# guzba/zippy

Measured on AMD Instinct MI355X. Metric: GiB/s uncompressed throughput (compress BestSpeed + uncompress), 4096x1 MiB batch, higher is better.
Workload: dtype u8

## Files before the change

zippy_amd/csrc/zh_l1_match.hip:

```cpp
#include <cstdlib>
#include <cstring>

#include "zh_common.h"
#include "zh_kprof.h"
#include "zh_tables.h"

namespace {
constexpr uint32_t kHashMul = 0x1e35a7bdu;
constexpr uint32_t kCntWords = 1024;
struct __attribute__((packed)) Bytes16 {
  uint32_t x, y, z, w;
};

}

template <bool kLdsTable>
__global__ __launch_bounds__(64) void zh_l1_match_kernel(const uint8_t* __restrict__ d_src,
                                                         ZhCompressArgs a, int huffman_only,
                                                         uint16_t* __restrict__ table_pool,
                                                         uint32_t* __restrict__ next_frag,
                                                         const uint32_t* __restrict__ order,
                                                         uint32_t* __restrict__ cost, uint32_t ticket_base) {
  __shared__ uint32_t s_hist[ZH_HIST_STRIDE];
  __shared__ uint32_t s_scr[kCntWords];
  __shared__ uint32_t s_bits[512];
  __shared__ uint32_t s_nmatch;
  uint32_t* const s_cover = s_scr;

  const unsigned lane = zh_lane();
  __shared__ uint16_t s_table_lds[kLdsTable ? 16384 : 2];
  uint16_t* const s_table = kLdsTable ? s_table_lds : table_pool + (size_t)blockIdx.x * 16384u;
  uint32_t taken = 0;
  for (uint32_t ticket = ticket_base + blockIdx.x; ticket < a.nfrags; taken++) {
  const uint32_t f = order ? order[ticket] : ticket;
  const uint64_t t_start = zh_clock();
  KPROF_DECL(16);
  const ZhFragDesc fd = a.frags[f];
  const uint32_t n = fd.len;
  const uint8_t* src = d_src + fd.src_off;
  uint16_t* m_pos = a.m_pos + (size_t)f * ZH_MAX_MATCHES_PER_FRAG;
  uint16_t* m_len = a.m_len + (size_t)f * ZH_MAX_MATCHES_PER_FRAG;
  uint16_t* m_off = a.m_off + (size_t)f * ZH_MAX_MATCHES_PER_FRAG;

  const uint32_t mis = (uint32_t)((uintptr_t)src & 3u);
  const uint32_t* asrc = reinterpret_cast<const uint32_t*>(src - mis);
  const uint32_t last_dw = n ? (n + mis - 1u) >> 2 : 0u;
  auto dw = [&](uint32_t i) -> uint32_t { return asrc[i < last_dw ? i : last_dw]; };
  auto ld32 = [&](uint32_t p) -> uint32_t {
    const uint32_t q = p + mis, i = q >> 2;
    return __builtin_amdgcn_alignbyte(dw(i + 1), dw(i), q);
  };
  for (uint32_t i = lane; i < ZH_HIST_STRIDE; i += 64) s_hist[i] = 0;
  for (uint32_t i = lane; i < kCntWords; i += 64) s_scr[i] = 0;

  uint32_t table_size = 256, shift = 24;
  while (table_size < 16384u && table_size < n) {
    table_size <<= 1;
    shift--;
  }
  const uint32_t e0 = (!huffman_only && n >= 4) ? (((ld32(0) * kHashMul) >> 17) & 1u) << 15 : 0u;
  for (uint32_t i = lane; i < 512; i += 64) s_bits[i] = 0;
  zh_wave_sync();
  KPROF_MARK(0);

  {
    uint32_t nm = 0;
    if (!huffman_only && n >= 15) {
      const uint32_t ip_limit = n - 15;
      uint32_t ip = 1;
      uint32_t K = 0;
      bool post = false;
      bool finished = false;
      while (!finished) {
        const bool dense = post || K < 32u;
        uint32_t pos, step, W0 = 0;
        if (dense) {
          W0 = post ? ip - 1u : ip;
          pos = W0 + lane;
          step = 1;
        } else {
          const uint32_t s = 32 + K, q = s >> 5, r = s & 31u, j = lane;
          uint32_t off = q * j;
          if (j > 32u - r) off += j - (32u - r);
          if (j > 64u - r) off += j - (64u - r);
          pos = ip + off;
          step = (s + j) >> 5;
        }
        const bool valid = pos + step <= ip_limit;
        if (!valid) pos = 1;
        Bytes16 av = {0, 0, 0, 0};
        if (valid) av = *reinterpret_cast<const Bytes16*>(src + pos);
        const uint32_t a0 = av.x, a1 = av.y, a2 = av.z, a3 = av.w;
        const uint32_t hp = a0 * kHashMul;
        const uint32_t h = hp >> shift, tag = (hp >> 17) & 1u;
        uint32_t oldw = e0;
        if (valid && ((s_bits[h >> 5] >> (h & 31u)) & 1u))
          oldw = kLdsTable ? (uint32_t)s_table[h]
                           : (uint32_t)__hip_atomic_load(s_table + h, __ATOMIC_RELAXED, __HIP_MEMORY_SCOPE_AGENT);
        const uint32_t old = oldw & 0x7fffu;
        const bool fetch = valid && (oldw >> 15) == tag;
        const uint32_t ck = (h & (kCntWords * 4u - 1u)) >> 2, cs = (h & 3u) * 8u;
        if (valid) atomicAdd(&s_scr[ck], 1u << cs);
        zh_wave_sync();
        Bytes16 qv = {0, 0, 0, 0};
        if (fetch) qv = *reinterpret_cast<const Bytes16*>(src + old);
        const uint32_t cnt = valid ? (s_scr[ck] >> cs) & 255u : 0u;
        zh_wave_sync();
        if (valid) s_scr[ck] = 0;
        const uint32_t x0 = fetch ? a0 ^ qv.x : 1u;
        const uint32_t x1 = a1 ^ qv.y;
        const uint32_t x2 = a2 ^ qv.z;
        const uint32_t x3 = a3 ^ qv.w;
        const uint32_t c0 = min(((uint32_t)__ffs((int)x0) - 1u) >> 3, 4u);
        const uint32_t c1 = min(((uint32_t)__ffs((int)x1) - 1u) >> 3, 4u);
        const uint32_t c2 = min(((uint32_t)__ffs((int)x2) - 1u) >> 3, 4u);
        const uint32_t c3 = min(((uint32_t)__ffs((int)x3) - 1u) >> 3, 4u);
        const uint32_t c23 = c2 + (c2 == 4u ? c3 : 0u);
        const uint32_t c123 = c1 + (c1 == 4u ? c23 : 0u);
        const uint32_t eqlen = c0 + (c0 == 4u ? c123 : 0u);

        const uint64_t V = __ballot(valid);
        const uint64_t H = __ballot(valid && x0 == 0);
        const uint64_t C = __ballot(cnt > 1u);
        uint64_t Cw = C;
        if (C && __popcll(C) <= 16) {
          Cw = 0;
          for (uint64_t cm = C; cm; cm &= cm - 1) {
            const uint32_t g = (uint32_t)__ffsll((long long)cm) - 1u;
            const uint32_t hg = __builtin_amdgcn_readlane(h, g);
            const bool same_h = valid && h == hg;
            if (__ballot(same_h) & ((1ull << g) - 1ull)) Cw |= 1ull << g;
          }
        }
        const uint32_t t = V == ~0ull ? 64u : (uint32_t)__ffsll((long long)~V) - 1u;

        KPROF_MARK(1);
        KPROF_COUNT(6, 1);
#ifndef ZH_EMU
        __builtin_amdgcn_s_setprio(1);
#endif
        uint64_t ins = post ? 1ull : 0ull;
        uint32_t i = post ? 1u : 0u;
        bool reprobe = post;
        uint32_t hop = 0x8000u;
        if (dense) {
          const uint64_t ev = (H | Cw) >> lane;
          const uint32_t d = ev ? (uint32_t)__ffsll((long long)ev) - 1u : 64u;
          const uint32_t info = eqlen | ((uint32_t)((Cw >> lane) & 1ull) << 5);
          const uint32_t gi = (uint32_t)__shfl((int)info, (int)((lane + d) & 63u), 64);
          if (d < 32u && gi < 16u) {
            const uint32_t g0 = lane + d, nx = g0 + gi;
            hop = g0 | 0x40u | (nx << 8) | ((d + 1u) << 16) | ((nx <= 64u ? nx - 1u : g0) << 22);
          } else if (!ev && lane >= 32u) {
            hop = 63u | (64u << 8);
          }
        }
        const uint32_t tt = ip_limit > W0 ? ip_limit - W0 : 0u;
        for (;;) {
          if (dense && i < 64u) {
            uint64_t sel = 0;
            uint32_t cur = zh_bcast(i), tv = 0x8000u;
            KPROF_MARK(3);
            bool go = true;
            if (!reprobe && K) {
              tv = __builtin_amdgcn_readlane(hop, cur);
              go = !(tv & 0x8000u) && (tv & 0x40u) && K + ((tv & 63u) - cur) <= 31u;
            }
            const uint32_t lim = zh_bcast(tt < 64u ? tt : 64u);
            if (go && cur < lim) {
#ifdef ZH_EMU
              do {
                tv = __builtin_amdgcn_readlane(hop, cur);
                if ((tv & 0x8040u) != 0x40u) break;
                const uint32_t g = tv & 63u, nxt = (tv >> 8) & 127u;
                sel |= 1ull << g;
                ins |= (~0ull << cur) & (~0ull >> (63u - g));
                ins |= 1ull << (nxt <= 64u ? nxt - 1u : g);
                cur = nxt;
              } while (cur < lim);
#else
              uint32_t t0, g, nxt;
              uint64_t m1;
              asm volatile(
                  "1:\n\t"
                  "v_readlane_b32 %[tv], %[hop], %[cur]\n\t"
                  "s_bitcmp1_b32 %[tv], 6\n\t"
                  "s_cbranch_scc0 2f\n\t"
                  "s_and_b32 %[g], %[tv], 63\n\t"
                  "s_bitset1_b64 %[sel], %[g]\n\t"
                  "s_bfe_u32 %[t0], %[tv], 0x60010\n\t"
                  "s_bfm_b64 %[m1], %[t0], %[cur]\n\t"
                  "s_or_b64 %[ins], %[ins], %[m1]\n\t"
                  "s_bfe_u32 %[t0], %[tv], 0x60016\n\t"
                  "s_bitset1_b64 %[ins], %[t0]\n\t"
                  "s_bfe_u32 %[cur], %[tv], 0x70008\n\t"
                  "s_cmp_lt_u32 %[cur], %[lim]\n\t"
                  "s_cbranch_scc1 1b\n\t"
                  "2:"
                  : [tv] "=&s"(tv), [cur] "+s"(cur), [sel] "+s"(sel), [ins] "+s"(ins), [t0] "=&s"(t0),
                    [g] "=&s"(g), [nxt] "=&s"(nxt), [m1] "=&s"(m1)
                  : [hop] "v"(hop), [lim] "s"(lim)
                  : "scc");
#endif
            }
            const bool chained = cur != i;
            bool run_out = false;
            if (go && cur < lim && !(tv & 0x8040u) && tt >= 64u) {
              K = (chained || reprobe ? 63u : K + 64u) - cur;
              ins |= ~0ull << cur;
              run_out = true;
            }
            KPROF_MARK(2);
            if (sel) {
              KPROF_COUNT(8, __popcll(sel));
              if ((sel >> lane) & 1ull) {
                const uint32_t k = nm + (uint32_t)__popcll(sel & zh_lanemask_lt());
                zh_store_nt(m_pos + k, (uint16_t)pos);
                zh_store_nt(m_len + k, (uint16_t)eqlen);
                zh_store_nt(m_off + k, (uint16_t)(pos - old));
              }
              nm += (uint32_t)__popcll(sel);
            }
            if (run_out) {
              post = false;
              ip = W0 + 64u;
              break;
            }
            if (chained) {
              K = 0;
              if (cur >= tt) {
                finished = true;
                break;
              }
              if (cur >= 64u) {
                post = true;
                ip = W0 + cur;
                break;
              }
              i = cur;
              reprobe = true;
            }
          }
          KPROF_COUNT(9, 1);
          if (i >= t) {
            finished = true;
            break;
          }
          uint32_t g = i;
          if (!reprobe) {
            const uint32_t last_dense = dense ? i + (31u - K) : 63u;
            uint32_t lim = last_dense < 63u ? last_dense : 63u;
            if (t - 1u < lim) lim = t - 1u;
            const uint64_t E = (H | Cw) & (~0ull << i);
            g = E ? (uint32_t)__ffsll((long long)E) - 1u : 64u;
            if (g > lim) {
              KPROF_COUNT(12, 1);
              ins |= (~0ull << i) & (~0ull >> (63u - lim));
              if (dense && lim == last_dense) {
                K = 32;
                ip = W0 + lim + 1u;
                post = false;
              } else if (lim + 1u == t && t < 64u) {
                finished = true;
              } else {
                K += 64u - i;
                post = false;
                if (dense) {
                  ip = W0 + 64u;
                } else {
                  ip = __builtin_amdgcn_readlane(pos, 63) + __builtin_amdgcn_readlane(step, 63);
                }
              }
              break;
            }
            if (g > i) ins |= (~0ull << i) & ((1ull << g) - 1ull);
            K += g - i;
          }
          uint32_t cand, flen;
          bool hit;
          if ((Cw >> g) & 1ull) {
            KPROF_COUNT(14, 1);
            const uint32_t hg = __builtin_amdgcn_readlane(h, g);
            const uint64_t same = __ballot(h == hg) & ins;
            if (same) {
              const uint32_t k = 63u - (uint32_t)__clzll((long long)same);
              cand = __builtin_amdgcn_readlane(pos, k);
              hit = __builtin_amdgcn_readlane(a0, k) == __builtin_amdgcn_readlane(a0, g);
              flen = 4;
              if (hit) {
                const uint32_t y1 = (uint32_t)__builtin_amdgcn_readlane(a1, k) ^ (uint32_t)__builtin_amdgcn_readlane(a1, g);
                if (y1) {
                  flen = 4u + (((uint32_t)__ffs((int)y1) - 1u) >> 3);
                } else {
                  const uint32_t y2 = (uint32_t)__builtin_amdgcn_readlane(a2, k) ^ (uint32_t)__builtin_amdgcn_readlane(a2, g);
                  if (y2) {
                    flen = 8u + (((uint32_t)__ffs((int)y2) - 1u) >> 3);
                  } else {
                    const uint32_t y3 = (uint32_t)__builtin_amdgcn_readlane(a3, k) ^ (uint32_t)__builtin_amdgcn_readlane(a3, g);
                    flen = y3 ? 12u + (((uint32_t)__ffs((int)y3) - 1u) >> 3) : 16u;
                  }
                }
              }
            } else {
              cand = __builtin_amdgcn_readlane(old, g);
              hit = (H >> g) & 1ull;
              flen = __builtin_amdgcn_readlane(eqlen, g);
            }
          } else {
            cand = __builtin_amdgcn_readlane(old, g);
            hit = (H >> g) & 1ull;
            flen = __builtin_amdgcn_readlane(eqlen, g);
          }
          ins |= 1ull << g;
          if (!hit) {
            if (reprobe) {
              reprobe = false;
              K = 0;
            } else {
              K++;
            }
            i = g + 1u;
            if (dense && K == 32u) {
              ip = W0 + i;
              post = false;
              break;
            }
            if (i >= 64u) {
              post = false;
              ip = dense ? W0 + 64u
                         : __builtin_amdgcn_readlane(pos, 63) + __builtin_amdgcn_readlane(step, 63);
              break;
            }
            continue;
          }
          const uint32_t mp = __builtin_amdgcn_readlane(pos, g);
          const uint32_t limit = n < mp + 258u ? n : mp + 258u;
          uint32_t matched;
          if (flen < 16u) {
            KPROF_COUNT(15, 1);
            matched = flen;
          } else {
            KPROF_COUNT(10, 1);
            zh_wave_sync();
            const uint32_t o = flen + 4u * lane;
            uint32_t avail = 0;
            if (mp + o < limit) avail = limit - (mp + o) < 4u ? limit - (mp + o) : 4u;
            const uint32_t x = ld32(mp + o) ^ ld32(cand + o);
            uint32_t eq = min(((uint32_t)__ffs((int)x) - 1u) >> 3, 4u);
            if (eq > avail) eq = avail;
            const uint64_t stop = __ballot(eq < 4u);
            const uint32_t fl = (uint32_t)__ffsll((long long)stop) - 1u;
            matched = flen + 4u * fl + __builtin_amdgcn_readlane(eq, fl);
          }
          if (matched > limit - mp) matched = limit - mp;
          if (lane == 0) {
            zh_store_nt(m_pos + nm, (uint16_t)mp);
            zh_store_nt(m_len + nm, (uint16_t)matched);
            zh_store_nt(m_off + nm, (uint16_t)(mp - cand));
          }
          nm++;
          ip = mp + matched;
          K = 0;
          post = true;
          if (ip >= ip_limit) {
            finished = true;
            break;
          }
          const uint32_t ni = g + matched;
          if (!dense || ni >= 64u) break;
          ins |= 1ull << (ni - 1u);
          i = ni;
          reprobe = true;
        }
        KPROF_MARK(3);
#ifndef ZH_EMU
        __builtin_amdgcn_s_setprio(0);
#endif
        if (finished) break;
        const bool mine = (ins >> lane) & 1ull;
        if (mine) atomicOr(&s_bits[h >> 5], 1u << (h & 31u));
        if (mine && !((C >> lane) & 1ull)) s_table[h] = (uint16_t)(pos | (tag << 15));
        uint64_t cc = ins & C;
        while (cc) {
          const uint32_t jx = (uint32_t)__ffsll((long long)cc) - 1u;
          cc &= cc - 1;
          if (lane == jx) s_table[h] = (uint16_t)(pos | (tag << 15));
        }
        zh_wave_sync();
        KPROF_MARK(4);
      }
    }
    if (lane == 0) s_nmatch = nm;
  }
  __threadfence_block();
  zh_wave_sync();
  KPROF_MARK(3);
  const uint32_t nmatch = s_nmatch;

  uint32_t extra_bits = 0, covered = 0;
  {
    const uint32_t mlast = nmatch ? nmatch - 1u : 0u;
    auto at = [&](uint32_t m) { return m < nmatch ? m : mlast; };
    uint32_t pq = m_pos[at(lane)], lq = m_len[at(lane)], oq = m_off[at(lane)];
    for (uint32_t m = lane; m - lane < nmatch; m += 64) {
      const uint32_t p = pq, l = lq, o = oq;
      pq = m_pos[at(m + 64u)];
      lq = m_len[at(m + 64u)];
      oq = m_off[at(m + 64u)];
      if (m < nmatch) {
        const uint32_t li = zh_len_code(l), di = zh_dist_code(o);
        atomicAdd(&s_hist[257 + li], 1u);
        atomicAdd(&s_hist[ZH_NUM_LITLEN + di], 1u);
        extra_bits += zh_len_extra_bits(li) + zh_dist_extra_bits(di);
        covered += l;
        atomicXor(&s_cover[(p + 1u) >> 5], 1u << ((p + 1u) & 31u));
        if (p + l < kCntWords * 32u) atomicXor(&s_cover[(p + l) >> 5], 1u << ((p + l) & 31u));
      }
    }
  }
  zh_wave_sync();
  {
    uint32_t carry = 0;
    for (uint32_t w0 = 0; w0 < kCntWords && w0 * 32u < n; w0 += 64) {
      uint32_t x = s_cover[w0 + lane];
#pragma unroll
      for (uint32_t sh = 1; sh < 32; sh <<= 1) x ^= x << sh;
      const uint64_t odd = __ballot((x >> 31) != 0u);
      if ((carry + (uint32_t)__popcll(odd & zh_lanemask_lt())) & 1u) x = ~x;
      s_cover[w0 + lane] = x;
      carry += (uint32_t)__popcll(odd);
    }
  }
  zh_wave_sync();
  if (a.f_cover) {
    uint32_t* cov_out = a.f_cover + (size_t)f * kCntWords;
    for (uint32_t w0 = 0; w0 * 32u < n; w0 += 64) cov_out[w0 + lane] = s_cover[w0 + lane];
  }
  for (uint32_t base = 0; base < n; base += 1024) {
    uint32_t wq[4];
#pragma unroll
    for (uint32_t u = 0; u < 4; u++) {
      const uint32_t p = base + 256u * u + 4u * lane;
      wq[u] = p < n ? ld32(p) : 0u;
    }
#pragma unroll
    for (uint32_t u = 0; u < 4; u++) {
      const uint32_t p = base + 256u * u + 4u * lane;
      if (p < n) {
        const uint32_t wi = p >> 5;
        const uint32_t c_lo = s_cover[wi], c_hi = wi + 1u < kCntWords ? s_cover[wi + 1u] : 0u;
        const uint32_t cov = (uint32_t)((((uint64_t)c_hi << 32) | c_lo) >> (p & 31u));
        const uint32_t notlit = cov | (cov >> 1);
#pragma unroll
        for (uint32_t k = 0; k < 4; k++)
          if (p + k < n && !((notlit >> k) & 1u)) atomicAdd(&s_hist[(wq[u] >> (8u * k)) & 255u], 1u);
      }
    }
  }
  extra_bits = zh_wave_sum(extra_bits);
  covered = zh_wave_sum(covered);
  zh_wave_sync();

  uint16_t* hist_out = a.f_hist + (size_t)f * ZH_HIST_STRIDE;
  for (uint32_t i = lane; i < ZH_HIST_STRIDE; i += 64) hist_out[i] = (uint16_t)s_hist[i];
  if (lane == 0) {
    a.f_nmatch[f] = nmatch;
    a.f_spill[f] = 0;
    a.f_nlit[f] = n - covered;
    a.f_extra_bits[f] = extra_bits;
  }
  KPROF_MARK(5);
  KPROF_COUNT(11, 1);
  KPROF_FLUSH(0, 16);
  zh_wave_sync();
  {
    uint32_t nf = 0;
    if (lane == 0) {
      if (cost) {
        const uint64_t dt = zh_clock() - t_start;
        cost[f] = dt < 0xffffffffull ? (uint32_t)dt : 0xffffffffu;
      }
      nf = atomicAdd(next_frag, 1u);
    }
    ticket = zh_bcast(nf);
  }
  }
  if (lane == 0 && taken) atomicAdd(next_frag + (kLdsTable ? 2 : 1), taken);
}

namespace {
constexpr uint32_t kCostClasses = 64;
__device__ __forceinline__ uint32_t cost_class(uint32_t c) {
  if (c < 1024u) return 0u;
  const uint32_t lg = 31u - (uint32_t)__clz((int)c);
  const uint32_t k = (lg - 10u) * 4u + ((c >> (lg - 2u)) & 3u);
  return k < kCostClasses ? k : kCostClasses - 1u;
}
}
__global__ __launch_bounds__(256) void zh_l1_cost_hist_kernel(const uint32_t* __restrict__ cost, uint32_t n,
                                                              uint32_t* __restrict__ hist) {
  __shared__ uint32_t s_h[kCostClasses];
  if (threadIdx.x < kCostClasses) s_h[threadIdx.x] = 0;
  __syncthreads();
  const uint32_t i = blockIdx.x * 256u + threadIdx.x;
  if (i < n) atomicAdd(&s_h[cost_class(cost[i])], 1u);
  __syncthreads();
  if (threadIdx.x < kCostClasses && s_h[threadIdx.x]) atomicAdd(&hist[threadIdx.x], s_h[threadIdx.x]);
}
__global__ __launch_bounds__(64) void zh_l1_cost_places_kernel(uint32_t* __restrict__ hist) {
  const unsigned lane = zh_lane();
  const uint32_t mine = hist[kCostClasses - 1u - lane];
  const uint32_t incl = zh_wave_scan(mine);
  hist[kCostClasses + (kCostClasses - 1u - lane)] = incl - mine;
}
__global__ __launch_bounds__(256) void zh_l1_cost_sort_kernel(const uint32_t* __restrict__ cost, uint32_t n,
                                                              uint32_t* __restrict__ hist, uint32_t* __restrict__ order) {
  const uint32_t i = blockIdx.x * 256u + threadIdx.x;
  if (i < n) order[atomicAdd(&hist[kCostClasses + cost_class(cost[i])], 1u)] = i;
}
__global__ __launch_bounds__(64) void zh_l1_cost_cut_kernel(uint32_t* __restrict__ hist, uint32_t tail) {
  const unsigned lane = zh_lane();
  const uint32_t incl = zh_wave_scan(hist[lane]);
  const uint64_t fits = __ballot(incl <= tail);
  const uint32_t k = (uint32_t)__popcll(fits);
  if (lane == 0) hist[kCostClasses] = k ? k - 1u : 0xffffffffu;
  if (lane == (k ? k - 1u : 0u)) hist[kCostClasses + 1u] = k ? incl : 0u;
}
__global__ __launch_bounds__(256) void zh_l1_cost_count_kernel(const uint32_t* __restrict__ cost, uint32_t n,
                                                               const uint32_t* __restrict__ hist,
                                                               uint32_t* __restrict__ blk) {
  const uint32_t i = blockIdx.x * 256u + threadIdx.x, cut = hist[kCostClasses];
  const bool last = i < n && cut != 0xffffffffu && cost_class(cost[i]) <= cut;
  const uint32_t c = (uint32_t)__popcll(__ballot(last));
  __shared__ uint32_t s_c[4];
  if (zh_lane() == 0) s_c[threadIdx.x >> 6] = c;
  __syncthreads();
  if (threadIdx.x == 0) blk[blockIdx.x] = s_c[0] + s_c[1] + s_c[2] + s_c[3];
}
__global__ __launch_bounds__(1024) void zh_l1_cost_scan_kernel(uint32_t* __restrict__ blk, uint32_t nblk) {
  __shared__ uint32_t s_w[16], s_carry;
  const uint32_t tid = threadIdx.x;
  if (tid == 0) s_carry = 0;
  __syncthreads();
  for (uint32_t base = 0; base < nblk; base += 1024u) {
    const uint32_t i = base + tid, v = i < nblk ? blk[i] : 0u;
    const uint32_t incl = zh_wave_scan(v);
    if (zh_lane() == 63) s_w[tid >> 6] = incl;
    __syncthreads();
    uint32_t before = s_carry;
    for (uint32_t w = 0; w < (tid >> 6); w++) before += s_w[w];
    if (i < nblk) blk[i] = before + incl - v;
    __syncthreads();
    if (tid == 1023) s_carry = before + incl;
    __syncthreads();
  }
}
__global__ __launch_bounds__(256) void zh_l1_cost_scatter_kernel(const uint32_t* __restrict__ cost, uint32_t n,
                                                                 const uint32_t* __restrict__ hist,
                                                                 const uint32_t* __restrict__ blk,
                                                                 uint32_t* __restrict__ order) {
  const uint32_t i = blockIdx.x * 256u + threadIdx.x, cut = hist[kCostClasses], ntail = hist[kCostClasses + 1u];
  const bool last = i < n && cut != 0xffffffffu && cost_class(cost[i]) <= cut;
  const uint64_t m = __ballot(last);
  __shared__ uint32_t s_c[4];
  if (zh_lane() == 0) s_c[threadIdx.x >> 6] = (uint32_t)__popcll(m);
  __syncthreads();
  uint32_t before = blk[blockIdx.x] + (uint32_t)__popcll(m & zh_lanemask_lt());
  for (uint32_t w = 0; w < (threadIdx.x >> 6); w++) before += s_c[w];
  if (i < n) order[last ? (n - ntail) + before : i - before] = i;
}

namespace {
long l1_slots_env() {
  static const long v = [] {
    const char* e = getenv("ZH_L1_SLOTS");
    const long v = e ? atol(e) : 0;
    return v >= 1 && v <= 16384 ? v : 0;
  }();
  return v;
}
uint32_t l1_lds_waves() {
  static const uint32_t waves = [] {
    const char* e = getenv("ZH_L1_LDS_WAVES");
    const long v = e ? atol(e) : -1;
    return v >= 0 && v <= 1024 ? (uint32_t)v : 256u;
  }();
  return waves;
}
}

extern "C" uint32_t zh_l1_table_slots(void) { return l1_slots_env() ? (uint32_t)l1_slots_env() : 4864u; }

__global__ void zh_l1_set_counter_kernel(uint32_t* next_frag, uint32_t v) {
  next_frag[0] = v;
  next_frag[1] = next_frag[2] = 0;
}

__global__ void zh_l1_head_start_kernel() {}

extern "C" ZhL1Launch zh_l1_match_prepare(hipStream_t stream, uint32_t nfrags, uint32_t* next_frag, uint32_t* cost,
                                          uint32_t* order, uint32_t* hist, int use_order, int side_ok) {
  ZhL1Launch l = {0, 0, nullptr};
  if (!nfrags) return l;
#ifdef ZH_XCHECK
  static const bool lds = [] {
    const char* e = getenv("ZH_L1_TABLE");
    return e && strcmp(e, "lds") == 0;
  }();
  if (lds) {
    l.lds = nfrags < 1024u ? nfrags : 1024u;
    hipLaunchKernelGGL(zh_l1_set_counter_kernel, dim3(1), dim3(1), 0, stream, next_frag, l.lds);
    return l;
  }
#endif
  const uint32_t mixed_pooled = l1_slots_env() ? (uint32_t)l1_slots_env() : 4096u;
  if (side_ok && l1_lds_waves() && nfrags >= mixed_pooled + l1_lds_waves()) {
    l.pooled = mixed_pooled;
    l.lds = l1_lds_waves();
  } else {
    l.pooled = nfrags < zh_l1_table_slots() ? nfrags : zh_l1_table_slots();
  }
  const uint32_t grid = l.pooled + l.lds;
  const bool sorted = use_order && cost && order && hist && nfrags > grid;
  if (sorted) {
    const uint32_t g = (nfrags + 255u) / 256u;
    static const uint32_t rounds = [] {
      const char* e = getenv("ZH_L1_TAIL_ROUNDS");
      const long v = e ? atol(e) : 0;
      return v >= 1 && v <= 64 ? (uint32_t)v : 2u;
    }();
    const uint32_t tail = nfrags / 2u < rounds * grid ? nfrags / 2u : rounds * grid;
    uint32_t* blk = hist + 128;
    (void)hipMemsetAsync(hist, 0, 128u * sizeof(uint32_t), stream);
    hipLaunchKernelGGL(zh_l1_cost_hist_kernel, dim3(g), dim3(256), 0, stream, cost, nfrags, hist);
    if (nfrags < 8u * grid) {
      hipLaunchKernelGGL(zh_l1_cost_places_kernel, dim3(1), dim3(64), 0, stream, hist);
      hipLaunchKernelGGL(zh_l1_cost_sort_kernel, dim3(g), dim3(256), 0, stream, cost, nfrags, hist, order);
    } else {
      hipLaunchKernelGGL(zh_l1_cost_cut_kernel, dim3(1), dim3(64), 0, stream, hist, tail);
      hipLaunchKernelGGL(zh_l1_cost_count_kernel, dim3(g), dim3(256), 0, stream, cost, nfrags, hist, blk);
      hipLaunchKernelGGL(zh_l1_cost_scan_kernel, dim3(1), dim3(1024), 0, stream, blk, g);
      hipLaunchKernelGGL(zh_l1_cost_scatter_kernel, dim3(g), dim3(256), 0, stream, cost, nfrags, hist, blk, order);
    }
    l.order = order;
  }
  hipLaunchKernelGGL(zh_l1_set_counter_kernel, dim3(1), dim3(1), 0, stream, next_frag, grid);
  return l;
}

extern "C" void zh_launch_l1_match(hipStream_t stream, const uint8_t* d_src, ZhCompressArgs a, int huffman_only,
                                   uint16_t* table_pool, uint32_t* next_frag, uint32_t* cost, ZhL1Launch l,
                                   int lds_part) {
  if (lds_part) {
    if (l.lds)
      hipLaunchKernelGGL(zh_l1_match_kernel<true>, dim3(l.lds), dim3(64), 0, stream, d_src, a, huffman_only, table_pool,
                         next_frag, l.order, cost, l.pooled);
  } else if (l.pooled) {
    static const uint32_t head_start = [] {
      const char* e = getenv("ZH_L1_HEAD_START");
      const long v = e ? atol(e) : -1;
      return v >= 0 && v <= 16 ? (uint32_t)v : 3u;
    }();
    for (uint32_t i = 0; l.lds && i < head_start; i++)
      hipLaunchKernelGGL(zh_l1_head_start_kernel, dim3(1), dim3(1), 0, stream);
    hipLaunchKernelGGL(zh_l1_match_kernel<false>, dim3(l.pooled), dim3(64), 0, stream, d_src, a, huffman_only,
                       table_pool, next_frag, l.order, cost, 0u);
  }
}
```

Baseline: 45.75.

## Shrink LDS footprint by aliasing parse maps and packing histogram counters

```diff
diff --git a/zippy_amd/csrc/zh_l1_match.hip b/zippy_amd/csrc/zh_l1_match.hip
--- a/zippy_amd/csrc/zh_l1_match.hip
+++ b/zippy_amd/csrc/zh_l1_match.hip
@@ -8,6 +8,10 @@
 namespace {
 constexpr uint32_t kHashMul = 0x1e35a7bdu;
 constexpr uint32_t kCntWords = 1024;
+constexpr uint32_t kBitsWords = 512, kFlagBits = 12, kFlagWords = (1u << kFlagBits) / 32u;
+static_assert(kBitsWords + 2u * kFlagWords <= kCntWords, "the parse's maps lie inside the coverage bitmap's words");
+constexpr uint32_t kHistWords = ZH_HIST_STRIDE / 2;
+static_assert(ZH_HIST_STRIDE % 2 == 0, "packed pairs");
 struct __attribute__((packed)) Bytes16 {
   uint32_t x, y, z, w;
 };
@@ -21,10 +25,12 @@
                                                          uint32_t* __restrict__ next_frag,
                                                          const uint32_t* __restrict__ order,
                                                          uint32_t* __restrict__ cost, uint32_t ticket_base) {
-  __shared__ uint32_t s_hist[ZH_HIST_STRIDE];
+  __shared__ uint32_t s_hist[kHistWords];
   __shared__ uint32_t s_scr[kCntWords];
-  __shared__ uint32_t s_bits[512];
   __shared__ uint32_t s_nmatch;
+  uint32_t* const s_bits = s_scr;
+  uint32_t* const s_seen = s_scr + kBitsWords;
+  uint32_t* const s_dup = s_seen + kFlagWords;
   uint32_t* const s_cover = s_scr;
 
   const unsigned lane = zh_lane();
@@ -50,16 +56,13 @@
     const uint32_t q = p + mis, i = q >> 2;
     return __builtin_amdgcn_alignbyte(dw(i + 1), dw(i), q);
   };
-  for (uint32_t i = lane; i < ZH_HIST_STRIDE; i += 64) s_hist[i] = 0;
-  for (uint32_t i = lane; i < kCntWords; i += 64) s_scr[i] = 0;
-
   uint32_t table_size = 256, shift = 24;
   while (table_size < 16384u && table_size < n) {
     table_size <<= 1;
     shift--;
   }
   const uint32_t e0 = (!huffman_only && n >= 4) ? (((ld32(0) * kHashMul) >> 17) & 1u) << 15 : 0u;
-  for (uint32_t i = lane; i < 512; i += 64) s_bits[i] = 0;
+  for (uint32_t i = lane; i < kBitsWords + 2u * kFlagWords; i += 64) s_scr[i] = 0;
   zh_wave_sync();
   KPROF_MARK(0);
 
@@ -99,14 +102,15 @@
                            : (uint32_t)__hip_atomic_load(s_table + h, __ATOMIC_RELAXED, __HIP_MEMORY_SCOPE_AGENT);
         const uint32_t old = oldw & 0x7fffu;
         const bool fetch = valid && (oldw >> 15) == tag;
-        const uint32_t ck = (h & (kCntWords * 4u - 1u)) >> 2, cs = (h & 3u) * 8u;
-        if (valid) atomicAdd(&s_scr[ck], 1u << cs);
-        zh_wave_sync();
+        const uint32_t ck = (h & ((1u << kFlagBits) - 1u)) >> 5, cb = 1u << (h & 31u);
+        const uint32_t seen_before = valid ? atomicOr(&s_seen[ck], cb) : 0u;
         Bytes16 qv = {0, 0, 0, 0};
         if (fetch) qv = *reinterpret_cast<const Bytes16*>(src + old);
-        const uint32_t cnt = valid ? (s_scr[ck] >> cs) & 255u : 0u;
+        if (seen_before & cb) atomicOr(&s_dup[ck], cb);
         zh_wave_sync();
-        if (valid) s_scr[ck] = 0;
+        const bool flagged = valid && (s_dup[ck] & cb);
+        zh_wave_sync();
+        if (valid) s_seen[ck] = s_dup[ck] = 0;
         const uint32_t x0 = fetch ? a0 ^ qv.x : 1u;
         const uint32_t x1 = a1 ^ qv.y;
         const uint32_t x2 = a2 ^ qv.z;
@@ -121,7 +125,7 @@
 
         const uint64_t V = __ballot(valid);
         const uint64_t H = __ballot(valid && x0 == 0);
-        const uint64_t C = __ballot(cnt > 1u);
+        const uint64_t C = __ballot(flagged);
         uint64_t Cw = C;
         if (C && __popcll(C) <= 16) {
           Cw = 0;
@@ -396,8 +400,12 @@
   zh_wave_sync();
   KPROF_MARK(3);
   const uint32_t nmatch = s_nmatch;
+  for (uint32_t i = lane; i < kCntWords; i += 64) s_scr[i] = 0;
+  for (uint32_t i = lane; i < kHistWords; i += 64) s_hist[i] = 0;
+  zh_wave_sync();
 
   uint32_t extra_bits = 0, covered = 0;
+  auto hist_add = [&](uint32_t sym) { atomicAdd(&s_hist[sym >> 1], 1u << (16u * (sym & 1u))); };
   {
     const uint32_t mlast = nmatch ? nmatch - 1u : 0u;
     auto at = [&](uint32_t m) { return m < nmatch ? m : mlast; };
@@ -409,8 +417,8 @@
       oq = m_off[at(m + 64u)];
       if (m < nmatch) {
         const uint32_t li = zh_len_code(l), di = zh_dist_code(o);
-        atomicAdd(&s_hist[257 + li], 1u);
-        atomicAdd(&s_hist[ZH_NUM_LITLEN + di], 1u);
+        hist_add(257u + li);
+        hist_add(ZH_NUM_LITLEN + di);
         extra_bits += zh_len_extra_bits(li) + zh_dist_extra_bits(di);
         covered += l;
         atomicXor(&s_cover[(p + 1u) >> 5], 1u << ((p + 1u) & 31u));
@@ -453,7 +461,7 @@
         const uint32_t notlit = cov | (cov >> 1);
 #pragma unroll
         for (uint32_t k = 0; k < 4; k++)
-          if (p + k < n && !((notlit >> k) & 1u)) atomicAdd(&s_hist[(wq[u] >> (8u * k)) & 255u], 1u);
+          if (p + k < n && !((notlit >> k) & 1u)) hist_add((wq[u] >> (8u * k)) & 255u);
       }
     }
   }
@@ -462,7 +470,7 @@
   zh_wave_sync();
 
   uint16_t* hist_out = a.f_hist + (size_t)f * ZH_HIST_STRIDE;
-  for (uint32_t i = lane; i < ZH_HIST_STRIDE; i += 64) hist_out[i] = (uint16_t)s_hist[i];
+  for (uint32_t i = lane; i < ZH_HIST_STRIDE; i += 64) hist_out[i] = (uint16_t)(s_hist[i >> 1] >> (16u * (i & 1u)));
   if (lane == 0) {
     a.f_nmatch[f] = nmatch;
     a.f_spill[f] = 0;
@@ -583,7 +591,7 @@
   static const uint32_t waves = [] {
     const char* e = getenv("ZH_L1_LDS_WAVES");
     const long v = e ? atol(e) : -1;
-    return v >= 0 && v <= 1024 ? (uint32_t)v : 256u;
+    return v >= 0 && v <= 1024 ? (uint32_t)v : 512u;
   }();
   return waves;
 }
```

Result: faster. 46.99 (median of 6 runs) (+2.7%).
